# generic-ebpf/generic-ebpf

Measured on AMD Instinct MI355X. Metric: Mpkt/s device-resident (64-insn filter, 64B pkts); achieved HBM GB/s vs peak, higher is better.
Workload: dtype u64; 1 GPU; c4; desc=64-insn classify + array-map lookup, 64 B packets, packets_total=67108864, packets_per_gpu=67108864, packet_bytes=64, prog_slots=553, dprog_entries=122, variant=0, exec=compiled, kernel_layout=staged64, parallelism=dp1, launch=eager, faulted_packets=0

## Files before the change

### generic-ebpf_amd/csrc/asm/gen_interp.py

```python
#!/usr/bin/env python3
import os
import re
import sys

NREG = 11
_NT = int(os.environ.get("EBPF_ASM_NT", "3"))
ST_POLICY = " nt" if _NT & 1 else ""
LD_POLICY = " nt" if _NT & 2 else ""
PROBE_POLICY = ""
for _v, _n in (("EBPF_ASM_STPOL", "ST_POLICY"), ("EBPF_ASM_LDPOL", "LD_POLICY"),
               ("EBPF_ASM_PROBEPOL", "PROBE_POLICY")):
    if os.environ.get(_v):
        _p = os.environ[_v].replace("+", " ")
        globals()[_n] = "" if _p == "none" else " " + _p
PKT0 = 22
V_PKT = 38
V_LEN = 40
V_T = 41
V_STK = 42
V_L16 = 43
V_IDX = 43
V_RES = 44
H = [46, 47, 48, 49, 50, 51]
R = list(range(52, 63))
# ... 4 lines not shown
assert RETK_STAGED in (1, 2, 4, 8)


STAGED_IMAGE = True

HIST_REPLICAS = 8
HIST_REPLICA_BYTES = 257 * 8
HIST_TICKET_OFF = HIST_REPLICAS * HIST_REPLICA_BYTES


def set_retk(k):
    global RETK, V_RB, NVGPR, SLOTS
    RETK = k
    V_RB = 44 if RETK == 1 else 64
    NVGPR = 64 if RETK == 1 else 64 + 2 * RETK
    SLOTS = 16 if RETK == 8 else RETK


set_retk(RETK_STAGED)

S_CB = 4
S_ENT = 8
S_ALIVE = 16
S_SAVE = 18
S_PROG, S_MAPS, S_DATA, S_OFFS, S_OFFBASE, S_RET, S_FAULTS, S_HIST = 20, 22, 24, 26, 28, 30, 32, 34
S_COUNT, S_STRIDE, S_START, S_NMAPS, S_NENT = 36, 38, 39, 40, 41
S_STKSTRIDE, S_LDSBASE = 42, 43
S_GROUP, S_GSTRIDE, S_NGROUPS, S_PKTLDS = 44, 45, 46, 47
S_MASK = 48
S_LINK = 50
S_CODE = 52
# ... 161 lines not shown
def mode_set(bit):
    return "s_or_b32 %s, %s, %s" % (s(S_MODE), s(S_MODE), "%d" % (1 << bit) if bit < 4 else "0x%x" % (1 << bit))


VF_OVERLAY = 0
VF_VSTORE = 1
VF_EXTENTS = 2
VF_KEEP = 3
VF_WCAP = 4
VF_ENTRIES_SHIFT, VF_ENTRIES_BITS = 8, 8
PKTLDS_HDRSTAGE = 31
PKTLDS_HDRKEEP = 30
WAVES_SB_SHIFT = 28
HIST_STORE = 0
WPHASE_PERIOD_SHIFT = 16
WPHASE_WIDE = 31

LOOP_BUDGET = 1 << 20
OVL_COUNT, VST_SCRATCH, WCOUNT, OVL_ENTRIES = 4, 8, 16, 24
WRITES_MAX = 16
FAULT_WRITES = 11


def variants(arity):
    if arity == 3:
        return [(d, o) for o in range(64) for d in range(NREG)]
    if arity == 2:
        return [(d, s) for d in range(NREG) for s in range(NREG)]
    if arity == 1:
        return [(d, None) for d in range(NREG)]
    return [(None, None)]
# ... 1743 lines not shown
              "s_mov_b64 exec, vcc",
              "s_mov_b32 m0, s67",
              "s_nop 0",
              "global_load_lds_dwordx4 %s, s[64:65]%s" % (v(H[4]), LD_POLICY)]
        if qq < 3:
            L += ["s_add_u32 s64, s64, 1024", "s_addc_u32 s65, s65, 0",
                  "s_add_u32 s67, s67, 1024"]
    L += [".Lpf_ret:",
          "s_setpc_b64 %s" % sp(S_LINK)]
    return L


def kernel(name, staged, jit=False):
    k = "K%s%s" % ("s" if staged else "g", "j" if jit else "")
    L = [".globl %s" % name, ".p2align 8", ".type %s,@function" % name, "%s:" % name]
    if name == "ebpf_jit_s64" and phased() and SLOTS == 16:
        L += [".globl ebpf_jit_s64w", ".type ebpf_jit_s64w,@function", "ebpf_jit_s64w:"]
    L += ["v_readfirstlane_b32 %s, v0" % s(S_WAVE),
          "s_lshr_b32 %s, %s, 6" % (s(S_WAVE), s(S_WAVE)),
          "s_load_dwordx16 s[%d:%d], %s" % (S_PROG, S_PROG + 15, karg_regs(
              ("prog", S_PROG), ("maps", S_MAPS), ("data", S_DATA), ("offsets", S_OFFS),
              ("off_base", S_OFFBASE), ("ret", S_RET), ("faults", S_FAULTS), ("hist", S_HIST))),
          "s_load_dwordx8 s[%d:%d], %s" % (S_COUNT, S_COUNT + 7, karg_regs(
              ("count", S_COUNT), ("stride", S_STRIDE), ("start", S_START), ("nmaps", S_NMAPS),
              ("nentries", S_NENT), ("stack_stride", S_STKSTRIDE), ("lds_stack_base", S_LDSBASE))),
          "s_load_dword %s, %s" % (s(S_GSTRIDE), karg("total_waves")),
          "s_load_dword %s, %s" % (s(S_PKTLDS), karg("lds_pkt_base")),
          "s_mov_b64 %s, src_shared_base" % sp(S_SHARED),
          "v_mov_b32 v%d, 0x00010203" % V_SEL,
          "s_getpc_b64 %s" % sp(S_CB),
          ".L%s_pc:" % k,
          "s_add_u32 %s, %s, .Lcb-.L%s_pc" % (s(S_CB), s(S_CB), k),
# ... 95 lines not shown


def ret_slot_write(x0, x1):
    return ["v_mov_b32 v%d, %s" % (V_RES, x0), "v_mov_b32 v%d, %s" % (V_RES + 1, x1)]


def phased():
    return STAGED_IMAGE and RETK > 1


def slot_commit():
    if RETK == 1:
        return []
    L = ["s_mov_b64 exec, -1",
         "s_and_b32 %s, %s, %s" % (s(S_BYTES), s(S_GROUP), s(S_KMASK))]
    if phased() and SLOTS == 16:
        L += ["s_cmp_eq_u32 %s, 0" % s(S_BYTES),
              "s_cbranch_scc0 .Lsc_half",
              "s_bitcmp1_b32 %s, %d" % (s(S_WPHASE), WPHASE_WIDE),
              "s_cbranch_scc0 .Lsc_half",
              "s_xor_b32 %s, %s, 0x80000000" % (s(S_PEND), s(S_PEND)),
              ".Lsc_half:",
              "s_lshr_b32 %s, %s, 28" % (s(S_T0), s(S_PEND)),
              "s_and_b32 %s, %s, 8" % (s(S_T0), s(S_T0)),
              "s_or_b32 %s, %s, %s" % (s(S_BYTES), s(S_BYTES), s(S_T0)),
              "s_bitset1_b32 %s, %s" % (s(S_PEND), s(S_BYTES))]
    elif phased():
        L.append("s_bitset1_b32 %s, %s" % (s(S_PEND), s(S_BYTES)))
    return L + [
            "s_lshl_b32 %s, %s, 1" % (s(S_BYTES), s(S_BYTES)),
            "s_set_gpr_idx_on %s, gpr_idx(DST)" % s(S_BYTES),
            "v_mov_b32 v%d, v%d" % (V_RB, V_RES),
            "v_mov_b32 v%d, v%d" % (V_RB + 1, V_RES + 1),
            "s_set_gpr_idx_off"]


def store_phased(tag, final):
    P = s(S_PEND)
    L = ["s_cmp_eq_u32 %s, 0" % s(S_WPHASE),
         "s_cbranch_scc1 .Lph_off_%s" % tag] + (
        ["s_waitcnt lgkmcnt(0)"] if not final else []) + [
         "s_and_b32 %s, %s, 0xffff" % (s(S_T0), P),
         "s_cbranch_scc0 .Lsp_none_%s" % tag]
    if not final:
        L += [
              "s_and_b32 %s, %s, %s" % (s(S_T0), s(S_GROUP), s(S_KMASK)),
              "s_lshr_b32 %s, %s, 28" % (s(S_T1), P),
              "s_and_b32 %s, %s, 8" % (s(S_T1), s(S_T1)),
              "s_cmp_eq_u32 %s, 0" % s(S_T0),
              "s_cbranch_scc0 .Lph_nf_%s" % tag,
              "s_bitcmp1_b32 %s, %d" % (s(S_WPHASE), WPHASE_WIDE),
              "s_cbranch_scc0 .Lph_nf_%s" % tag,
              "s_xor_b32 %s, %s, 8" % (s(S_T1), s(S_T1)),
              ".Lph_nf_%s:" % tag,
              "s_or_b32 %s, %s, %s" % (s(S_T0), s(S_T0), s(S_T1)),
              "s_bitcmp1_b32 %s, %s" % (P, s(S_T0)),
              "s_cbranch_scc1 .Lph_write_%s" % tag,
              "s_and_b32 %s, %s, 0x%x" % (s(S_T1), s(S_WPHASE), 0x1f << WPHASE_PERIOD_SHIFT),
              "s_and_b32 %s, %s, 0xffff" % (s(S_T2), s(S_WPHASE)),
              "s_bfe_u32 %s, %s, %s" % (s(S_T0), s(S_CLOCK), s(S_T1)),
              "s_cmp_lt_u32 %s, %s" % (s(S_T0), s(S_T2)),
              "s_cbranch_scc0 .Lsp_none_%s" % tag,
              ".Lph_write_%s:" % tag]
    L += ["s_mov_b64 exec, -1",
          "v_lshrrev_b32 %s, 1, v%d" % (v(R[0]), V_L16),
          "s_andn2_b32 %s, %s, %s" % (s(S_T1), s(S_PREVG), s(S_KMASK)),
          "s_add_u32 %s, %s, %s" % (s(S_T2), s(S_GSTRIDE), s(S_KMASK)),
          "s_sub_u32 %s, %s, %s" % (s(S_T0), s(S_T1), s(S_T2)),
          "s_bitcmp1_b32 %s, %d" % (s(S_WPHASE), WPHASE_WIDE),
          "s_cselect_b32 %s, %s, 0" % (s(S_T2), s(S_T2)),
          "s_sub_u32 %s, %s, %s" % (s(S_T2), s(S_T0), s(S_T2)),
          "s_and_b32 %s, %s, %s" % (s(S_T3), s(S_PREVG), s(S_KMASK)),
          "s_lshr_b32 s66, %s, 6" % s(S_COUNT),
          "s_add_u32 s67, %s, %s" % (s(S_T1), s(S_KMASK)),
          "s_cmp_lt_u32 s67, s66",
          "s_cbranch_scc0 .Lph_ragged_%s" % tag]
    for lo, g in ((60, S_T1), (62, S_T0), (64, S_T2)):
        L += ["s_lshl_b32 s%d, %s, 9" % (lo, s(g)),
              "s_lshr_b32 s%d, %s, 23" % (lo + 1, s(g)),
              "s_add_u32 s%d, s%d, %s" % (lo, lo, s(S_RET)),
              "s_addc_u32 s%d, s%d, %s" % (lo + 1, lo + 1, s(S_RET + 1))]
    halves = [0] if RETK == SLOTS else [0, 1]

    def slots_of(half, ragged):
        out = []
        for own in (True, False):
            h = half if own else 1 - half
            if h not in halves:
                continue
            for i in range(RETK):
                j = 8 * h + i
                sk = ".Lph_%s%d_%d_%s" % ("r" if ragged else "f", half, j, tag)
                out += ["s_bitcmp1_b32 %s, %d" % (P, j), "s_cbranch_scc0 %s" % sk]
                if not ragged:
                    if own:
                        out += ["s_cmp_ge_u32 %s, %d" % (s(S_T3), i),
                                "s_cselect_b64 s[66:67], s[60:61], s[64:65]"]
                    out.append("global_store_dwordx2 %s, v[%d:%d], s[%d:%d] offset:%d%s" % (
                        v(R[0]), V_RB + 2 * j, V_RB + 2 * j + 1, 66 if own else 62,
                        67 if own else 63, 512 * i, ST_POLICY))
                else:
                    if own:
                        out += ["s_cmp_ge_u32 %s, %d" % (s(S_T3), i),
                                "s_cselect_b32 %s, %s, %s" % (s(S_BYTES), s(S_T1), s(S_T2))]
                    else:
                        out.append("s_mov_b32 %s, %s" % (s(S_BYTES), s(S_T0)))
                    out += ["s_add_u32 %s, %s, %d" % (s(S_BYTES), s(S_BYTES), i),
                            "s_lshl_b32 s66, %s, 6" % s(S_BYTES),
                            "s_sub_u32 s66, %s, s66" % s(S_COUNT),
                            "v_cmp_gt_u32_e64 vcc, s66, %s" % v(R[1]),
                            "s_mov_b64 exec, vcc",
                            "s_lshl_b32 s66, %s, 9" % s(S_BYTES),
                            "s_lshr_b32 s67, %s, 23" % s(S_BYTES),
                            "s_add_u32 s66, s66, %s" % s(S_RET),
                            "s_addc_u32 s67, s67, %s" % s(S_RET + 1),
                            "global_store_dwordx2 %s, v[%d:%d], s[66:67]%s" % (
                                v(R[0]), V_RB + 2 * j, V_RB + 2 * j + 1, ST_POLICY),
                            "s_mov_b64 exec, -1"]
                out.append(sk + ":")
        return out

    for ragged in (False, True):
        if ragged:
            L += [".Lph_ragged_%s:" % tag,
                  "v_lshrrev_b32 %s, 4, v%d" % (v(R[1]), V_L16)]
        if len(halves) > 1:
            L += ["s_bitcmp1_b32 %s, 31" % P,
                  "s_cbranch_scc1 .Lph_%sh1_%s" % ("r" if ragged else "f", tag)]
        L += slots_of(0, ragged) + ["s_branch .Lph_done_%s" % tag]
        if len(halves) > 1:
            L += [".Lph_%sh1_%s:" % ("r" if ragged else "f", tag)] + slots_of(1, ragged) + [
                  "s_branch .Lph_done_%s" % tag]
    L += [".Lph_done_%s:" % tag,
          "s_and_b32 %s, %s, 0x80000000" % (P, P),
          "s_branch .Lsp_none_%s" % tag,
          ".Lph_off_%s:" % tag]
    return L


def store_prev_results(tag, final):
    L = store_phased(tag, final) if phased() else []
    L += ["s_cmp_eq_u32 %s, -1" % s(S_PREVG),
         "s_cbranch_scc1 .Lsp_none_%s" % tag]
    if not final and RETK > 1:
        L += ["s_and_b32 %s, %s, %s" % (s(S_T0), s(S_PREVG), s(S_KMASK)),
              "s_cmp_lg_u32 %s, %s" % (s(S_T0), s(S_KMASK)),
              "s_cbranch_scc1 .Lsp_none_%s" % tag]
    L += ["s_mov_b64 exec, -1",
          "s_andn2_b32 %s, %s, %s" % (s(S_T0), s(S_PREVG), s(S_KMASK)) if RETK > 1 else
# ... 522 lines not shown
             ("L16", V_L16), ("RES", V_RES), ("GIDX", V_GIDX), ("HVAL", V_HVAL), ("SEL", V_SEL)]
    vregs += [("H%d" % i, r) for i, r in enumerate(H)] + [("R%d" % i, r) for i, r in enumerate(R)]
    out += ["#define AH_S_%s %d" % x for x in sregs] + ["#define AH_V_%s %d" % x for x in vregs]
    out += ["// bits of the mode word s[AH_S_MODE]"]
    out += ["#define AH_MODE_%s %d" % x for x in (
        ("STAGED", MODE_STAGED), ("JIT", MODE_JIT), ("STRUCTURED", MODE_STRUCTURED),
        ("HDRSTAGE", MODE_HDRSTAGE), ("OVERLAY", MODE_OVERLAY), ("KEEP", MODE_KEEP),
        ("EXTENTS", MODE_EXTENTS))]
    out += ["// dprog.h / ebpf_gpu.h values the kernels were generated with; asm_runtime.cpp asserts them"]
    values = (
        ("DP_VF_OVERLAY", 1 << VF_OVERLAY), ("DP_VF_VSTORE", 1 << VF_VSTORE),
        ("DP_VF_EXTENTS", 1 << VF_EXTENTS), ("DP_VF_KEEP", 1 << VF_KEEP), ("DP_VF_WCAP", 1 << VF_WCAP),
        ("DP_VF_ENTRIES_SHIFT", VF_ENTRIES_SHIFT), ("DP_VF_ENTRIES_MAX", (1 << VF_ENTRIES_BITS) - 1),
        ("DP_PKTLDS_HDRSTAGE", 1 << PKTLDS_HDRSTAGE), ("DP_PKTLDS_HDRKEEP", 1 << PKTLDS_HDRKEEP),
        ("DP_WAVES_SB_SHIFT", WAVES_SB_SHIFT), ("DP_HIST_STORE", 1 << HIST_STORE),
        ("DP_WPHASE_PERIOD_SHIFT", WPHASE_PERIOD_SHIFT), ("DP_WPHASE_WIDE", 1 << WPHASE_WIDE),
        ("DP_LOOP_BUDGET", LOOP_BUDGET), ("DP_OVL_COUNT", OVL_COUNT), ("DP_OVL_SCRATCH", VST_SCRATCH),
        ("DP_WCOUNT", WCOUNT), ("DP_OVL_ENTRIES", OVL_ENTRIES), ("DP_WRITES_MAX", WRITES_MAX),
        ("EBPF_FAULT_WRITES", FAULT_WRITES), ("DP_HIST_REPLICAS", HIST_REPLICAS),
        ("DP_HIST_REPLICA_BYTES", HIST_REPLICA_BYTES), ("DP_HIST_TICKET_OFF", HIST_TICKET_OFF),
        ("DP_HIST_PARTIAL_BYTES", HIST_TICKET_OFF + 64 * (HIST_REPLICAS + 1)))
    out += ["#define AH_%s %du" % x for x in values]
    out += ["#define AH_SHARED_VALUES(X) " + " ".join("X(%s)" % n for n, _ in values)]
    out += ["// ebpf_jit_tmpl's entries, in the table's order"]
    jt = [re.sub(r"^(\.Ljt_|\.Lr_|\.L|ebpf_)", "", n).upper() for n in JT_LABELS] + ["AREA_BYTES"]
    out += ["enum {"] + ["\tAH_JT_%s," % n for n in jt] + ["\tAH_JT_COUNT", "};"]
    out += ["#define AH_JIT_ENTRY_OFF %d  // a compiled program's start block in ebpf_jit_area" % JIT_ENTRY_OFF]
    return out


NSGPR_INTERP = S_JOIN
# ... 10 lines not shown
                                     (out_s0, 1, False, False),
                                     (out_s3, RETK_INTERP, True, True)):
        set_retk(k)
        INTERP_IMAGE = interp
        if not staged:
            NVGPR += GEN_HOIST_REGS
        h = generate(out_s, staged)
        header = header or h
        assert h[:-2] == header[:-2]
    header = header[:-2] + ["#define AH_RET_GROUPS_STAGED %d  // groups per result burst, staged kernels"
                            % RETK_STAGED,
                            "#define AH_NVGPR_STAGED %d" % (64 if RETK_STAGED == 1 else 64 + 2 * RETK_STAGED),
                            "#define AH_RET_GROUPS_GENERAL 1",
                            "#define AH_NVGPR_STAGED_WIDE %d  // ebpf_jit_s64w: 16 result slots "
                            "(write phasing), 0 = none" % (96 if RETK_STAGED == 8 else 0),
                            "#define AH_NVGPR_GENERAL %d" % (64 + GEN_HOIST_REGS),
                            "#define AH_NVGPR_INTERP %d  // the interpreter's staged image (m3)"
                            % (64 if RETK_INTERP == 1 else 64 + 2 * RETK_INTERP),
                            "#define AH_RET_GROUPS_INTERP %d" % RETK_INTERP]
    with open(out_h, "w") as f:
        f.write("\n".join(header) + "\n")


def header_families():
    classes = []
    for _, _, cls, _ in FAMILIES:
        if cls not in classes:
            classes.append(cls)
    for cls in classes:
        idx = [i for _, _, c, i in FAMILIES if c == cls]
# ... 92 lines not shown
    header.append("#define AH_S_RUNMASK %d  // general image: s[76:77], a hoisted-load run's lanes" % S_RUNMASK)
    header.append("#define AH_V_IDX %d  // general image: the lane's packet index" % V_IDX)
    header.append("#define AH_RET_GROUPS %d" % RETK)
    header.append("#define AH_NVGPR %d" % NVGPR)
    A += link_kernel()
    A += [".p2align 2", ".Lhandler_table:"]
    A += ["  .long %s-.Llink_base" % lab for lab in table]
    A += [".p2align 2", "ebpf_jit_meta:"] + meta
    A += jit_templates()
    A += [".p2align 8", "ebpf_jit_area:", "  .fill %d, 4, 0xbf810000" % (JIT_AREA_BYTES // 4)]
    vtop = 0
    for ln in A:
        code = ln.split(";")[0].split("//")[0]
        for a, b, c in re.findall(r"\bv(\d+)\b|\bv\[(\d+):(\d+)\]", code):
            vtop = max(vtop, int(a or c))
    vwide = V_RB + 2 * SLOTS if (staged_image and SLOTS == 16) else NVGPR
    assert vtop < max(NVGPR, vwide), "image code uses v%d, the kernels allocate %d VGPRs" % (
        vtop, max(NVGPR, vwide))
    kernarg = 232
    nsg = NSGPR_STAGED if (staged_image or GEN_JOIN) else NSGPR_GEN
    if INTERP_IMAGE:
        top = 0
        for ln in A:
            for a, b, c in re.findall(r"\bs(\d+)\b|\bs\[(\d+):(\d+)\]", ln.split(";")[0].split("//")[0]):
                top = max(top, int(a or c))
        assert top < NSGPR_INTERP, "interpreter image uses s%d" % top
    ks = [("ebpf_interp_s64", kernarg, 0, NVGPR, NSGPR_INTERP if INTERP_IMAGE else nsg, 256),
          ("ebpf_interp_gen", kernarg, 0, NVGPR, nsg, 256),
          ("ebpf_jit_s64", kernarg, 0, NVGPR, nsg, 256),
          ("ebpf_jit_gen", kernarg, 0, NVGPR, nsg, 256),
          ("ebpf_asm_link", 16, 0, 16, 16, 64)]
    if vwide > NVGPR:
        ks.append(("ebpf_jit_s64w", kernarg, 0, vwide, nsg, 256))
    for name, ka, lds, vg, sg, wg in ks:
        A += kd(name, lds, vg, sg, ka, wg)
    md = metadata(ks)
    with open(out_s, "w") as f:
        f.write("\n".join(("\t" + x if not (x.endswith(":") or x.startswith(".") or x.startswith(" ")) else x)
                          for x in A) + "\n")
        f.write("\n".join(md) + "\n")
    return header


if __name__ == "__main__":
    main()
```

### generic-ebpf_amd/csrc/dprog.h

```cpp
#pragma once
#include <stdint.h>
#include <stddef.h>

enum dp_kind : uint16_t {
	DK_FAULT = 0x100,
	DK_CALL_LOOKUP = 0x101,
	DK_MOV64R = 0x102,
	DK_NEG64 = 0x103,
	DK_NEG32 = 0x104,
	DK_ARSH64I = 0x105,
	DK_ARSH64R = 0x106,
	DK_ARSH32I = 0x107,
	DK_ARSH32R = 0x108,
	DK_DIV64Z = 0x109,
	DK_MOD64Z = 0x10a,
	DK_DIV32Z = 0x10b,
	DK_MOD32Z = 0x10c,
	DK_CALL_UPDATE = 0x10d,
	DK_LOOPINIT = 0x10e,
	DK_LOOPCNT = 0x10f,
	DK_CALL_HDELETE = 0x110,
	DK_CNT_STORE = 0x111,
	DK_XADD = 0x112,
	DK_OVLINIT = 0x113,
};
#define DP_VF_OVERLAY 1u
#define DP_VF_VSTORE 2u
#define DP_VF_EXTENTS 4u
#define DP_VF_KEEP 8u
#define DP_VF_WCAP 16u
#define DP_VF_ENTRIES_SHIFT 8u
#define DP_VF_ENTRIES_MAX 255u
#define DP_PKTLDS_HDRSTAGE 0x80000000u
#define DP_PKTLDS_HDRKEEP 0x40000000u
#define DP_WAVES_SB_SHIFT 28u
#define DP_HIST_STORE 1u
#define DP_WPHASE_PERIOD_SHIFT 16u
#define DP_WPHASE_WIDE 0x80000000u
#define DP_AUX_SIZE 0xffu
#define DP_AUX_FETCH 0x100u
#define DP_AUX_IMM 0x200u
#define DP_AUX_SYNTH 1u
#define DP_AUX_DELETE 1u
#define DP_LOOP_BUDGET (1u << 20)
#define DP_CLS_JMP32 6

struct dp_entry {
	uint64_t handler;
	uint64_t imm;
	uint32_t next;
	uint32_t target;
	uint16_t kind;
	uint8_t dst, src;
// ... 94 lines not shown
```

### generic-ebpf_amd/csrc/host/asm_jit.cpp

```cpp
#include <elf.h>
#include <hip/hip_runtime.h>

#include "asm_cc.h"
#include "asm_handlers.h"
#include "gfx950_enc.h"
#include "runtime.h"

int asm_lower(const dprog_host &xl, int mode, const std::vector<dp_map> &table,
	      std::vector<dp_entry> &out, uint32_t *stack_stride, std::string *err);

namespace {

static_assert(AH_S_OPND == 10 && AH_JT_MOV_S11 == AH_JT_MOV_S10 + 1 && AH_JT_MOV_S12 == AH_JT_MOV_S10 + 2 &&
		      AH_JT_MOV_S13 == AH_JT_MOV_S10 + 3 && AH_JT_MOV_S14 == AH_JT_MOV_S10 + 4 &&
		      AH_JT_MOV_S15 == AH_JT_MOV_S10 + 5,
	      "the s_mov templates of the operand registers s10..s15 are consecutive");

struct jit_image {
	bool ok = false;
	std::string why;
	size_t cb = 0;
	std::vector<uint32_t> body_off, body_len;
	uint32_t t[AH_JT_COUNT] = {};
};
// ... 564 lines not shown
		}
		memcpy(&img[area + pos[e]], g.data(), g.size());
	}
	if (structured) {
		g.clear();
		G.long_jump(T[AH_JT_GROUP_DONE]);
		memcpy(&img[area + end_pos], g.data(), g.size());
	}
	if (code)
		code->assign(img.begin() + area, img.begin() + area + total);
	return 0;
}

int
asm_jit_build(int device, const dprog_host &xl, int mode, const std::vector<dp_map> &table,
	      void **mod_out, void **fn_out, void **fn_wide_out, uint32_t *stack_stride,
	      std::string *err)
{
	std::vector<unsigned char> img;
	int e = asm_jit_emit(xl, mode, table, &img, nullptr, stack_stride, err);
	if (e)
		return e;
	if (hipSetDevice(device) != hipSuccess)
		return EIO;
	hipModule_t mod = nullptr;
	if (hipModuleLoadData(&mod, img.data()) != hipSuccess) {
		*err = "loading the compiled program failed";
		return EIO;
	}
	hipFunction_t fn = nullptr;
	if (hipModuleGetFunction(&fn, mod, mode == 1 ? "ebpf_jit_s64" : "ebpf_jit_gen") != hipSuccess) {
		hipModuleUnload(mod);
		*err = "compiled program kernel missing";
		return EIO;
	}
	hipFunction_t fw = nullptr;
	if (fn_wide_out && mode == 1 && AH_NVGPR_STAGED_WIDE &&
	    hipModuleGetFunction(&fw, mod, "ebpf_jit_s64w") != hipSuccess)
		fw = nullptr;
	*mod_out = mod;
	*fn_out = fn;
	if (fn_wide_out)
		*fn_wide_out = fw;
	return 0;
}

void
asm_jit_release(void *mod)
{
	if (mod)
		hipModuleUnload(static_cast<hipModule_t>(mod));
}
```

### generic-ebpf_amd/csrc/host/asm_runtime.cpp

```cpp
#include <cstdio>
#include <hip/hip_runtime.h>

#include <algorithm>

#include "asm_handlers.h"
#include "runtime.h"

extern "C" hipError_t hipExtModuleLaunchKernel(hipFunction_t f, uint32_t gx, uint32_t gy, uint32_t gz,
					       uint32_t lx, uint32_t ly, uint32_t lz, size_t shared,
					       hipStream_t stream, void **params, void **extra,
					       hipEvent_t start, hipEvent_t stop, uint32_t flags);

#define X(member, off) \
	static_assert(offsetof(dp_launch, member) == off, \
		      "dp_launch." #member " is not where the kernels load it: " #off);
AH_LAUNCH_FIELDS(X)
#undef X
static_assert(sizeof(dp_launch) == AH_KERNARG_BYTES, "dp_launch is the kernels' argument block");
static_assert(offsetof(dp_map, handle) == AH_M_HANDLE && offsetof(dp_map, dev_base) == AH_M_DEV_BASE &&
		      offsetof(dp_map, value_size) == AH_M_VALUE_SIZE &&
		      offsetof(dp_map, max_entries) == AH_M_MAX_ENTRIES &&
		      offsetof(dp_map, lds_off) == AH_M_LDS_OFF && offsetof(dp_map, flags) == AH_M_FLAGS &&
		      sizeof(dp_map) == AH_MAP_REC_BYTES,
	      "dp_map is loaded whole into the kernels' record registers");
// ... 747 lines not shown
		lo = std::min(lo, x.handler);
		hi = std::max(hi, x.handler);
	}
	for (const dp_entry &x : back)
		if (x.handler == 0 || (x.handler & 3) || hi - lo > asm_image_len(mode)) {
			hipFree(d);
			*err = "handler link produced implausible addresses";
			return EIO;
		}
	*d_out = d;
	return 0;
}

hipError_t
launch_interp_asm(const dp_launch &L0, hipStream_t stream, int device, int mode,
		  uint32_t map_lds_bytes, void *fn, void *fn_wide, uint32_t stream_cap, hipEvent_t ev_start,
		  hipEvent_t ev_stop, unsigned long long *user_hist, bool hist_overwrite)
{
	asm_module *mod = module_for(device);
	if (!mod->ok)
		return hipErrorNotSupported;
	const uint64_t chunk = 1ull << 28;
	for (uint64_t c0 = 0; c0 < L0.count; c0 += chunk) {
		dp_launch L = L0;
		L.count = (L0.count - c0 < chunk) ? L0.count - c0 : chunk;
		if (L0.offsets)
			L.offsets = L0.offsets + ((L0.vflags & DP_VF_EXTENTS) ? 2 * c0 : c0);
		else
			L.data = L0.data + c0 * L0.stride;
		L.ret = L0.ret + c0;
		L.pkt_base = L0.pkt_base + c0;
		if (L0.faults)
// ... 32 lines not shown
		uint32_t sb = retk;
		if (interp_staged)
			sb = kInterpSuperblock;
		if (const char *ks = getenv("EBPF_SUPERBLOCK"))
			while (sb > 1 && (uint32_t)atoi(ks) < sb)
				sb >>= 1;
		uint64_t wgs = (groups + 4 * sb - 1) / (4 * sb);
		if (wgs > cap)
			wgs = cap;
		uint32_t log2k = 0;
		while ((1u << log2k) < sb)
			log2k++;
		L.total_waves = (uint32_t)(wgs * 4) | (log2k << DP_WAVES_SB_SHIFT);
		L.wphase = 0;
		if (mode == 1 && !interp_staged && sb > 1 && stream_cap == kStreamWorkgroups &&
		    groups >= 2 * sb * 4 * wgs)
			L.wphase = fn_wide ? (DP_WPHASE_WIDE | (12u << DP_WPHASE_PERIOD_SHIFT) | 1024u)
					   : ((11u << DP_WPHASE_PERIOD_SHIFT) | 640u);
		if (const char *wp = getenv("EBPF_WPHASE")) {
			unsigned bits = 0, win = 0, slots = 8;
			const int nf = sscanf(wp, "%u,%u,%u", &bits, &win, &slots);
			L.wphase = (nf >= 2 && bits >= 4 && bits <= 20 && win < (1u << bits))
				       ? ((bits << DP_WPHASE_PERIOD_SHIFT) | win) : 0u;
			if (L.wphase && slots == 16 && fn_wide)
				L.wphase |= DP_WPHASE_WIDE;
			if (!(mode == 1 && !interp_staged && sb > 1))
				L.wphase = 0;
		}
		if ((L.wphase & DP_WPHASE_WIDE) && fn_wide && AH_NVGPR_STAGED_WIDE) {
			const uint64_t wide_cap = (uint64_t)mod->cus * std::min<uint32_t>(
				wg_per_cu, 512 / ((AH_NVGPR_STAGED_WIDE + 7) & ~7));
			if (wgs > wide_cap) {
				wgs = wide_cap;
				L.total_waves = (uint32_t)(wgs * 4) | (log2k << DP_WAVES_SB_SHIFT);
			}
		}
		L.hist_user = user_hist;
		L.hist_flags = (hist_overwrite && c0 == 0) ? DP_HIST_STORE : 0u;
		L.nwg = (uint32_t)wgs;
		size_t sz = sizeof(L);
		void *extra[] = {HIP_LAUNCH_PARAM_BUFFER_POINTER, &L, HIP_LAUNCH_PARAM_BUFFER_SIZE, &sz,
				 HIP_LAUNCH_PARAM_END};
		hipFunction_t k = fn ? static_cast<hipFunction_t>((L.wphase & DP_WPHASE_WIDE) ? fn_wide : fn)
				     : (mode == 1 ? mod->k_staged : mod->k_general);
		if (L.hist && !L.hist_rows)
			return hipErrorInvalidValue;
		const bool single = c0 == 0 && L0.count <= chunk;
		hipError_t e;
		if (single && ev_start && ev_stop) {
			e = hipExtModuleLaunchKernel(k, (uint32_t)wgs * 256u, 1, 1, 256, 1, 1, lds, stream,
						     nullptr, extra, ev_start, ev_stop, 0);
		} else {
			if (ev_start && c0 == 0)
				hipEventRecord(ev_start, stream);
			e = hipModuleLaunchKernel(k, (unsigned)wgs, 1, 1, 256, 1, 1, lds, stream, nullptr,
						  extra);
			if (e == hipSuccess && ev_stop && c0 + chunk >= L0.count)
				hipEventRecord(ev_stop, stream);
// ... 30 lines not shown
```

### generic-ebpf_amd/csrc/host/gpu_runtime.cpp

```cpp
#include <chrono>

#include "runtime.h"

namespace {

uint32_t
plan_map_lds(const struct ebpf_map *em, uint32_t *used)
{
	if (em->is_hashtable())
		return ~0u;
	const uint64_t bytes = (uint64_t)em->value_size * em->max_entries;
	if (bytes == 0 || bytes % 4 != 0 || *used + bytes > kMapLdsBudget)
		return ~0u;
	const uint32_t off = kMapLdsBase + *used;
	*used += (uint32_t)((bytes + 15) & ~15ull);
	return off;
}

dp_map
map_record(const struct ebpf_map *em, uint32_t *lds_used)
{
	const map_device_layout l = map_device_layout_of(em);
	dp_map m;
	memset(&m, 0, sizeof(m));
// ... 167 lines not shown
	return 0;
}

static int
jit_entries(struct ebpf_prog *ep, dprog_device *dp, int mode)
{
	std::lock_guard<std::mutex> g(ep->dlock);
	if (dp->jit_fn[mode])
		return 0;
	if (dp->jit_err[mode])
		return dp->jit_err[mode];
	std::string msg;
	const auto t0 = std::chrono::steady_clock::now();
	int err = asm_jit_build(dp->device, *ep->xlated, mode, dp->table, &dp->jit_mod[mode],
				&dp->jit_fn[mode], mode == 1 ? &dp->jit_fn_wide : nullptr,
				&dp->jit_stride[mode], &msg);
	dp->build_ms[mode] =
	    std::chrono::duration<double, std::milli>(std::chrono::steady_clock::now() - t0).count();
	if (err) {
		dp->jit_err[mode] = err;
		return fail(err, msg);
	}
	return 0;
}

static int
asm_entries(struct ebpf_prog *ep, dprog_device *dp, int mode)
{
	std::lock_guard<std::mutex> g(ep->dlock);
	if (dp->d_asm[mode])
// ... 93 lines not shown
		unsigned long long *user_hist = L.hist;
		if (L.hist) {
			void *part = nullptr;
			if ((err = rows_acquire(dp->device, stream, &part)))
				return fail(err, "no verdict-partial buffer");
			L.hist_rows = static_cast<uint32_t *>(part);
			L.hist = static_cast<unsigned long long *>(part);
		}
		bool hash = false;
		for (const dp_map &m : dp->table)
			hash = hash || (m.flags & DP_MAP_HASH) != 0;
		uint32_t wg_cap = 0;
		if (mode == 1 && fn)
			wg_cap = (hash || ep->xlated->has_loops) ? kProbeWorkgroups : kStreamWorkgroups;
		e = launch_interp_asm(L, stream, dp->device, mode, dp->map_lds_bytes, fn,
				      fn ? dp->jit_fn_wide : nullptr, wg_cap, ev_start, ev_stop, user_hist,
				      hist_overwrite);
	} else {
		L.prog = dp->d_entries;
		dp->last_exec = EBPF_EXEC_HIP;
		dp->last_layout = 0;
		if (hist_overwrite && L.hist &&
		    (e = hipMemsetAsync(L.hist, 0, EBPF_HIST_BINS * sizeof(uint64_t), stream)) !=
			hipSuccess)
			return hip_fail(e, "hipMemsetAsync(hist)");
		if (spill) {
			const uint64_t per = 16ull * ep->xlated->ovl_entries;
			uint64_t chunk = std::max<uint64_t>(256, ((1ull << 30) / per) & ~255ull);
			chunk = std::min<uint64_t>(chunk, std::max<uint64_t>(L.count, 1));
			uint8_t *buf = nullptr;
			if ((err = ovl_acquire(dp->device, stream, chunk * per, &buf)))
// ... 240 lines not shown
```

### generic-ebpf_amd/csrc/host/internal.h

```cpp
#pragma once

#include <errno.h>
#include <stdint.h>
#include <stdlib.h>
#include <string.h>

#include <atomic>
#include <memory>
#include <mutex>
#include <set>
#include <string>
#include <vector>

#include "ebpf.h"
#include "ebpf_gpu.h"
#include "ebpf_vm_isa.h"
#include "../dprog.h"
#include "map_writes.h"

#define EBPF_EXPORT extern "C" __attribute__((visibility("default")))

enum ebpf_obj_type_id : uint32_t { EBPF_OBJ_TYPE_PROG = 0, EBPF_OBJ_TYPE_MAP = 1 };

struct ebpf_env {
// ... 74 lines not shown

struct dprog_device {
	int device = -1;
	dp_entry *d_entries = nullptr;
	dp_map *d_maps = nullptr;
	std::vector<dp_map> table;
	uint32_t nentries = 0;
	uint32_t nmaps = 0;
	uint32_t map_lds_bytes = 0;
	dp_entry *d_asm[kModes] = {};
	uint32_t asm_stride[kModes] = {};
	int asm_err[kModes] = {};
	void *jit_mod[kModes] = {};
	void *jit_fn[kModes] = {};
	void *jit_fn_wide = nullptr;
	uint32_t jit_stride[kModes] = {};
	int jit_err[kModes] = {};
	double build_ms[kModes] = {};
	void *d_upd = nullptr;
	std::vector<struct upd_map> upd_host;
	uint64_t win_words = 0;
	uint32_t upd_stride = 0;
	int last_exec = -1;
	int last_layout = -1;
};

struct dprog_host;
bool prog_writes_maps(const dprog_host &xl);

enum av_kind : uint8_t {
// ... 86 lines not shown
```

### generic-ebpf_amd/csrc/host/runtime.h

```cpp
#pragma once
#include <hip/hip_runtime.h>

#include <algorithm>

#include "internal.h"

int fail(int err, const std::string &msg);
int hip_fail(hipError_t e, const char *what);
int device_count();
void take_time_events(hipEvent_t *start, hipEvent_t *stop);

inline bool
in_list(const std::vector<uint16_t> &v, size_t t)
{
	return std::find(v.begin(), v.end(), (uint16_t)t) != v.end();
}

struct rows_slot;
struct upd_owner {
	rows_slot *slot = nullptr;
	unsigned long long sid = 0;
};
int rows_acquire(int device, hipStream_t stream, void **out);
int ovl_acquire(int device, hipStream_t stream, size_t bytes, uint8_t **out);
// ... 41 lines not shown
int upd_plan_for(struct ebpf_prog *ep, dprog_device *dp, uint64_t count, hipStream_t stream, upd_plan *P);
int upd_fetch(const dprog_device *dp, const upd_plan &P, hipStream_t stream, uint64_t first, host_log *out);
int upd_apply_host(struct ebpf_prog *ep, const std::vector<host_log> &logs, bool arrays);
int delta_merge_host(struct ebpf_prog *ep, int ndev, const int *devices);
int upd_finish(struct ebpf_prog *ep, dprog_device *dp, const upd_plan &P, hipStream_t stream);

int prepare(struct ebpf_prog *ep, int device, dprog_device **out);
int launch(struct ebpf_prog *ep, dprog_device *dp, const dp_launch &L0, hipStream_t stream,
	   hipEvent_t ev_start = nullptr, hipEvent_t ev_stop = nullptr, bool hist_overwrite = false,
	   upd_plan *plan = nullptr);
int validate_batch(const struct ebpf_pkt_batch *b, uint32_t allowed_flags = 0);
int check_device(int device);

hipError_t launch_interp_v0(const dp_launch &L, hipStream_t stream);
hipError_t launch_interp_asm(const dp_launch &L, hipStream_t stream, int device, int mode,
			     uint32_t map_lds_bytes, void *fn, void *fn_wide, uint32_t stream_cap,
			     hipEvent_t ev_start, hipEvent_t ev_stop, unsigned long long *user_hist,
			     bool hist_overwrite);
int asm_available(int device);
bool asm_lds_fits(int mode, uint32_t map_lds_bytes, uint32_t stack_stride);
bool asm_program_needs_general(const dprog_host &xl);
bool asm_program_stores_last(const dprog_host &xl);
bool asm_program_gstage(const dprog_host &xl);
bool asm_program_hdrlds(const dprog_host &xl);
bool asm_hdrlds_fits(uint32_t map_lds_bytes, uint32_t stack_stride);
int asm_build_entries(int device, const dprog_host &xl, int mode, const std::vector<dp_map> &table,
		      dp_entry **d_out, uint32_t *stack_stride, std::string *err);
int asm_jit_build(int device, const dprog_host &xl, int mode, const std::vector<dp_map> &table,
		  void **mod_out, void **fn_out, void **fn_wide_out, uint32_t *stack_stride, std::string *err);
void asm_jit_release(void *mod);
int asm_jit_emit(const dprog_host &xl, int mode, const std::vector<dp_map> &table,
		 std::vector<unsigned char> *img_out, std::vector<unsigned char> *code,
		 uint32_t *stack_stride, std::string *err);
int rccl_hist_allreduce(int ndev, const int *devices, uint64_t *const *hist, hipStream_t *streams,
			std::string *msg);
```

Before: 87880 Mpkt/s.

## Add 32-slot result write phasing kernel variant for staged JIT

Extends the write-phasing scheme for result stores from 16 to 32 buffered result slots, organised as four rotating quarters tracked by a cursor field in the wphase word. A new ebpf_jit_s64x entry point with 128 VGPRs is emitted and selected by the host when there are enough groups, using a longer period and window. The aim is to batch more result writes into larger, less frequent bursts to reduce HBM write interference. The cost is higher VGPR pressure, which caps workgroups per CU and lowers occupancy, plus more scalar bookkeeping per commit.

```diff
diff --git a/generic-ebpf_amd/csrc/asm/gen_interp.py b/generic-ebpf_amd/csrc/asm/gen_interp.py
--- a/generic-ebpf_amd/csrc/asm/gen_interp.py
+++ b/generic-ebpf_amd/csrc/asm/gen_interp.py
@@ -42,7 +42,7 @@
     RETK = k
     V_RB = 44 if RETK == 1 else 64
     NVGPR = 64 if RETK == 1 else 64 + 2 * RETK
-    SLOTS = 16 if RETK == 8 else RETK
+    SLOTS = 32 if RETK == 8 else RETK
 
 
 set_retk(RETK_STAGED)
@@ -234,7 +234,10 @@
 WAVES_SB_SHIFT = 28
 HIST_STORE = 0
 WPHASE_PERIOD_SHIFT = 16
-WPHASE_WIDE = 31
+WPHASE_CUR_SHIFT = 24
+WPHASE_HQ_SHIFT = 30
+WPHASE_WIDE = 1 << WPHASE_HQ_SHIFT
+WPHASE_X32 = 3 << WPHASE_HQ_SHIFT
 
 LOOP_BUDGET = 1 << 20
 OVL_COUNT, VST_SCRATCH, WCOUNT, OVL_ENTRIES = 4, 8, 16, 24
@@ -2008,8 +2011,9 @@
 def kernel(name, staged, jit=False):
     k = "K%s%s" % ("s" if staged else "g", "j" if jit else "")
     L = [".globl %s" % name, ".p2align 8", ".type %s,@function" % name, "%s:" % name]
-    if name == "ebpf_jit_s64" and phased() and SLOTS == 16:
-        L += [".globl ebpf_jit_s64w", ".type ebpf_jit_s64w,@function", "ebpf_jit_s64w:"]
+    if name == "ebpf_jit_s64" and phased() and SLOTS > RETK:
+        L += [".globl ebpf_jit_s64w", ".type ebpf_jit_s64w,@function", "ebpf_jit_s64w:",
+              ".globl ebpf_jit_s64x", ".type ebpf_jit_s64x,@function", "ebpf_jit_s64x:"]
     L += ["v_readfirstlane_b32 %s, v0" % s(S_WAVE),
           "s_lshr_b32 %s, %s, 6" % (s(S_WAVE), s(S_WAVE)),
           "s_load_dwordx16 s[%d:%d], %s" % (S_PROG, S_PROG + 15, karg_regs(
@@ -2135,15 +2139,17 @@
         return []
     L = ["s_mov_b64 exec, -1",
          "s_and_b32 %s, %s, %s" % (s(S_BYTES), s(S_GROUP), s(S_KMASK))]
-    if phased() and SLOTS == 16:
+    if phased() and SLOTS > RETK:
         L += ["s_cmp_eq_u32 %s, 0" % s(S_BYTES),
-              "s_cbranch_scc0 .Lsc_half",
-              "s_bitcmp1_b32 %s, %d" % (s(S_WPHASE), WPHASE_WIDE),
-              "s_cbranch_scc0 .Lsc_half",
-              "s_xor_b32 %s, %s, 0x80000000" % (s(S_PEND), s(S_PEND)),
-              ".Lsc_half:",
-              "s_lshr_b32 %s, %s, 28" % (s(S_T0), s(S_PEND)),
-              "s_and_b32 %s, %s, 8" % (s(S_T0), s(S_T0)),
+              "s_cbranch_scc0 .Lsc_quarter",
+              "s_lshr_b32 %s, %s, %d" % (s(S_T0), s(S_WPHASE), WPHASE_HQ_SHIFT),
+              "s_lshl_b32 %s, %s, %d" % (s(S_T0), s(S_T0), WPHASE_CUR_SHIFT),
+              "s_or_b32 %s, %s, 0x%x" % (s(S_T0), s(S_T0), 0xffffffff & ~(7 << WPHASE_CUR_SHIFT)),
+              "s_add_u32 %s, %s, 0x%x" % (s(S_WPHASE), s(S_WPHASE), 1 << WPHASE_CUR_SHIFT),
+              "s_and_b32 %s, %s, %s" % (s(S_WPHASE), s(S_WPHASE), s(S_T0)),
+              ".Lsc_quarter:",
+              "s_bfe_u32 %s, %s, 0x%x" % (s(S_T0), s(S_WPHASE), 2 << 16 | WPHASE_CUR_SHIFT),
+              "s_lshl_b32 %s, %s, %d" % (s(S_T0), s(S_T0), RETK.bit_length() - 1),
               "s_or_b32 %s, %s, %s" % (s(S_BYTES), s(S_BYTES), s(S_T0)),
               "s_bitset1_b32 %s, %s" % (s(S_PEND), s(S_BYTES))]
     elif phased():
@@ -2158,22 +2164,23 @@
 
 def store_phased(tag, final):
     P = s(S_PEND)
+    cur_field = 2 << 16 | WPHASE_CUR_SHIFT
     L = ["s_cmp_eq_u32 %s, 0" % s(S_WPHASE),
          "s_cbranch_scc1 .Lph_off_%s" % tag] + (
         ["s_waitcnt lgkmcnt(0)"] if not final else []) + [
-         "s_and_b32 %s, %s, 0xffff" % (s(S_T0), P),
-         "s_cbranch_scc0 .Lsp_none_%s" % tag]
+         "s_cmp_eq_u32 %s, 0" % P,
+         "s_cbranch_scc1 .Lsp_none_%s" % tag]
     if not final:
         L += [
               "s_and_b32 %s, %s, %s" % (s(S_T0), s(S_GROUP), s(S_KMASK)),
-              "s_lshr_b32 %s, %s, 28" % (s(S_T1), P),
-              "s_and_b32 %s, %s, 8" % (s(S_T1), s(S_T1)),
+              "s_bfe_u32 %s, %s, 0x%x" % (s(S_T1), s(S_WPHASE), cur_field),
               "s_cmp_eq_u32 %s, 0" % s(S_T0),
               "s_cbranch_scc0 .Lph_nf_%s" % tag,
-              "s_bitcmp1_b32 %s, %d" % (s(S_WPHASE), WPHASE_WIDE),
-              "s_cbranch_scc0 .Lph_nf_%s" % tag,
-              "s_xor_b32 %s, %s, 8" % (s(S_T1), s(S_T1)),
+              "s_add_u32 %s, %s, 1" % (s(S_T1), s(S_T1)),
+              "s_lshr_b32 %s, %s, %d" % (s(S_T2), s(S_WPHASE), WPHASE_HQ_SHIFT),
+              "s_and_b32 %s, %s, %s" % (s(S_T1), s(S_T1), s(S_T2)),
               ".Lph_nf_%s:" % tag,
+              "s_lshl_b32 %s, %s, %d" % (s(S_T1), s(S_T1), RETK.bit_length() - 1),
               "s_or_b32 %s, %s, %s" % (s(S_T0), s(S_T0), s(S_T1)),
               "s_bitcmp1_b32 %s, %s" % (P, s(S_T0)),
               "s_cbranch_scc1 .Lph_write_%s" % tag,
@@ -2187,73 +2194,72 @@
           "v_lshrrev_b32 %s, 1, v%d" % (v(R[0]), V_L16),
           "s_andn2_b32 %s, %s, %s" % (s(S_T1), s(S_PREVG), s(S_KMASK)),
           "s_add_u32 %s, %s, %s" % (s(S_T2), s(S_GSTRIDE), s(S_KMASK)),
-          "s_sub_u32 %s, %s, %s" % (s(S_T0), s(S_T1), s(S_T2)),
-          "s_bitcmp1_b32 %s, %d" % (s(S_WPHASE), WPHASE_WIDE),
-          "s_cselect_b32 %s, %s, 0" % (s(S_T2), s(S_T2)),
-          "s_sub_u32 %s, %s, %s" % (s(S_T2), s(S_T0), s(S_T2)),
           "s_and_b32 %s, %s, %s" % (s(S_T3), s(S_PREVG), s(S_KMASK)),
+          "s_bfe_u32 s68, %s, 0x%x" % (s(S_WPHASE), cur_field),
+          "s_lshr_b32 s69, %s, %d" % (s(S_WPHASE), WPHASE_HQ_SHIFT),
+          "s_add_u32 %s, s69, 1" % s(S_BYTES),
+          "s_mul_i32 %s, %s, %s" % (s(S_BYTES), s(S_BYTES), s(S_T2)),
           "s_lshr_b32 s66, %s, 6" % s(S_COUNT),
           "s_add_u32 s67, %s, %s" % (s(S_T1), s(S_KMASK)),
           "s_cmp_lt_u32 s67, s66",
           "s_cbranch_scc0 .Lph_ragged_%s" % tag]
-    for lo, g in ((60, S_T1), (62, S_T0), (64, S_T2)):
-        L += ["s_lshl_b32 s%d, %s, 9" % (lo, s(g)),
-              "s_lshr_b32 s%d, %s, 23" % (lo + 1, s(g)),
-              "s_add_u32 s%d, s%d, %s" % (lo, lo, s(S_RET)),
-              "s_addc_u32 s%d, s%d, %s" % (lo + 1, lo + 1, s(S_RET + 1))]
-    halves = [0] if RETK == SLOTS else [0, 1]
-
-    def slots_of(half, ragged):
-        out = []
-        for own in (True, False):
-            h = half if own else 1 - half
-            if h not in halves:
-                continue
-            for i in range(RETK):
-                j = 8 * h + i
-                sk = ".Lph_%s%d_%d_%s" % ("r" if ragged else "f", half, j, tag)
-                out += ["s_bitcmp1_b32 %s, %d" % (P, j), "s_cbranch_scc0 %s" % sk]
-                if not ragged:
-                    if own:
-                        out += ["s_cmp_ge_u32 %s, %d" % (s(S_T3), i),
-                                "s_cselect_b64 s[66:67], s[60:61], s[64:65]"]
-                    out.append("global_store_dwordx2 %s, v[%d:%d], s[%d:%d] offset:%d%s" % (
-                        v(R[0]), V_RB + 2 * j, V_RB + 2 * j + 1, 66 if own else 62,
-                        67 if own else 63, 512 * i, ST_POLICY))
-                else:
-                    if own:
-                        out += ["s_cmp_ge_u32 %s, %d" % (s(S_T3), i),
-                                "s_cselect_b32 %s, %s, %s" % (s(S_BYTES), s(S_T1), s(S_T2))]
-                    else:
-                        out.append("s_mov_b32 %s, %s" % (s(S_BYTES), s(S_T0)))
-                    out += ["s_add_u32 %s, %s, %d" % (s(S_BYTES), s(S_BYTES), i),
-                            "s_lshl_b32 s66, %s, 6" % s(S_BYTES),
-                            "s_sub_u32 s66, %s, s66" % s(S_COUNT),
-                            "v_cmp_gt_u32_e64 vcc, s66, %s" % v(R[1]),
-                            "s_mov_b64 exec, vcc",
-                            "s_lshl_b32 s66, %s, 9" % s(S_BYTES),
-                            "s_lshr_b32 s67, %s, 23" % s(S_BYTES),
-                            "s_add_u32 s66, s66, %s" % s(S_RET),
-                            "s_addc_u32 s67, s67, %s" % s(S_RET + 1),
-                            "global_store_dwordx2 %s, v[%d:%d], s[66:67]%s" % (
-                                v(R[0]), V_RB + 2 * j, V_RB + 2 * j + 1, ST_POLICY),
-                            "s_mov_b64 exec, -1"]
-                out.append(sk + ":")
-        return out
-
+    lg = RETK.bit_length() - 1
+
+    def quarter(h, ragged):
+        rf = "r" if ragged else "f"
+        out = ["s_bfe_u32 s66, %s, 0x%x" % (P, RETK << 16 | RETK * h),
+               "s_cbranch_scc0 .Lph_%sq%d_%s" % (rf, h, tag),
+               "s_sub_u32 s64, s68, %d" % h,
+               "s_and_b32 s64, s64, s69",
+               "s_mul_i32 s65, s64, %s" % s(S_T2),
+               "s_sub_u32 %s, %s, s65" % (s(S_T0), s(S_T1)),
+               "s_cmp_eq_u32 s64, 0",
+               "s_cselect_b32 s65, %s, 0" % s(S_BYTES),
+               "s_cselect_b32 s64, %s, %d" % (s(S_T3), RETK - 1),
+               "s_sub_u32 s65, %s, s65" % s(S_T0)]
+        if not ragged:
+            for lo, g in ((60, s(S_T0)), (62, "s65")):
+                out += ["s_lshl_b32 s%d, %s, 9" % (lo, g),
+                        "s_lshr_b32 s%d, %s, 23" % (lo + 1, g),
+                        "s_add_u32 s%d, s%d, %s" % (lo, lo, s(S_RET)),
+                        "s_addc_u32 s%d, s%d, %s" % (lo + 1, lo + 1, s(S_RET + 1))]
+        for i in range(RETK):
+            j = RETK * h + i
+            sk = ".Lph_%s%d_%s" % (rf, j, tag)
+            out += ["s_bitcmp1_b32 %s, %d" % (P, j), "s_cbranch_scc0 %s" % sk,
+                    "s_cmp_ge_u32 s64, %d" % i]
+            if not ragged:
+                out += ["s_cselect_b64 s[66:67], s[60:61], s[62:63]",
+                        "global_store_dwordx2 %s, v[%d:%d], s[66:67] offset:%d%s" % (
+                            v(R[0]), V_RB + 2 * j, V_RB + 2 * j + 1, 512 * i, ST_POLICY)]
+            else:
+                out += ["s_cselect_b32 s66, %s, s65" % s(S_T0),
+                        "s_add_u32 s66, s66, %d" % i,
+                        "s_lshl_b32 s67, s66, 6",
+                        "s_sub_u32 s67, %s, s67" % s(S_COUNT),
+                        "v_cmp_gt_u32_e64 vcc, s67, %s" % v(R[1]),
+                        "s_mov_b64 exec, vcc",
+                        "s_lshr_b32 s67, s66, 23",
+                        "s_lshl_b32 s66, s66, 9",
+                        "s_add_u32 s66, s66, %s" % s(S_RET),
+                        "s_addc_u32 s67, s67, %s" % s(S_RET + 1),
+                        "global_store_dwordx2 %s, v[%d:%d], s[66:67]%s" % (
+                            v(R[0]), V_RB + 2 * j, V_RB + 2 * j + 1, ST_POLICY),
+                        "s_mov_b64 exec, -1"]
+            out.append(sk + ":")
+        return out + [".Lph_%sq%d_%s:" % (rf, h, tag)]
+
+    assert 1 << lg == RETK and SLOTS % RETK == 0 and SLOTS <= 32
     for ragged in (False, True):
         if ragged:
             L += [".Lph_ragged_%s:" % tag,
                   "v_lshrrev_b32 %s, 4, v%d" % (v(R[1]), V_L16)]
-        if len(halves) > 1:
-            L += ["s_bitcmp1_b32 %s, 31" % P,
-                  "s_cbranch_scc1 .Lph_%sh1_%s" % ("r" if ragged else "f", tag)]
-        L += slots_of(0, ragged) + ["s_branch .Lph_done_%s" % tag]
-        if len(halves) > 1:
-            L += [".Lph_%sh1_%s:" % ("r" if ragged else "f", tag)] + slots_of(1, ragged) + [
-                  "s_branch .Lph_done_%s" % tag]
+        for h in range(SLOTS // RETK):
+            L += quarter(h, ragged)
+        if not ragged:
+            L.append("s_branch .Lph_done_%s" % tag)
     L += [".Lph_done_%s:" % tag,
-          "s_and_b32 %s, %s, 0x80000000" % (P, P),
+          "s_mov_b32 %s, 0" % P,
           "s_branch .Lsp_none_%s" % tag,
           ".Lph_off_%s:" % tag]
     return L
@@ -2806,7 +2812,8 @@
         ("DP_VF_ENTRIES_SHIFT", VF_ENTRIES_SHIFT), ("DP_VF_ENTRIES_MAX", (1 << VF_ENTRIES_BITS) - 1),
         ("DP_PKTLDS_HDRSTAGE", 1 << PKTLDS_HDRSTAGE), ("DP_PKTLDS_HDRKEEP", 1 << PKTLDS_HDRKEEP),
         ("DP_WAVES_SB_SHIFT", WAVES_SB_SHIFT), ("DP_HIST_STORE", 1 << HIST_STORE),
-        ("DP_WPHASE_PERIOD_SHIFT", WPHASE_PERIOD_SHIFT), ("DP_WPHASE_WIDE", 1 << WPHASE_WIDE),
+        ("DP_WPHASE_PERIOD_SHIFT", WPHASE_PERIOD_SHIFT), ("DP_WPHASE_WIDE", WPHASE_WIDE),
+        ("DP_WPHASE_X32", WPHASE_X32),
         ("DP_LOOP_BUDGET", LOOP_BUDGET), ("DP_OVL_COUNT", OVL_COUNT), ("DP_OVL_SCRATCH", VST_SCRATCH),
         ("DP_WCOUNT", WCOUNT), ("DP_OVL_ENTRIES", OVL_ENTRIES), ("DP_WRITES_MAX", WRITES_MAX),
         ("EBPF_FAULT_WRITES", FAULT_WRITES), ("DP_HIST_REPLICAS", HIST_REPLICAS),
@@ -2847,6 +2854,8 @@
                             "#define AH_RET_GROUPS_GENERAL 1",
                             "#define AH_NVGPR_STAGED_WIDE %d  // ebpf_jit_s64w: 16 result slots "
                             "(write phasing), 0 = none" % (96 if RETK_STAGED == 8 else 0),
+                            "#define AH_NVGPR_STAGED_X32 %d  // ebpf_jit_s64x: 32 result slots, 0 = none"
+                            % (128 if RETK_STAGED == 8 else 0),
                             "#define AH_NVGPR_GENERAL %d" % (64 + GEN_HOIST_REGS),
                             "#define AH_NVGPR_INTERP %d  // the interpreter's staged image (m3)"
                             % (64 if RETK_INTERP == 1 else 64 + 2 * RETK_INTERP),
@@ -2969,9 +2978,10 @@
         code = ln.split(";")[0].split("//")[0]
         for a, b, c in re.findall(r"\bv(\d+)\b|\bv\[(\d+):(\d+)\]", code):
             vtop = max(vtop, int(a or c))
-    vwide = V_RB + 2 * SLOTS if (staged_image and SLOTS == 16) else NVGPR
-    assert vtop < max(NVGPR, vwide), "image code uses v%d, the kernels allocate %d VGPRs" % (
-        vtop, max(NVGPR, vwide))
+    vwide = V_RB + 4 * RETK if (staged_image and SLOTS > RETK) else NVGPR
+    vx32 = V_RB + 2 * SLOTS if (staged_image and SLOTS > RETK) else NVGPR
+    assert vtop < max(NVGPR, vx32), "image code uses v%d, the kernels allocate %d VGPRs" % (
+        vtop, max(NVGPR, vx32))
     kernarg = 232
     nsg = NSGPR_STAGED if (staged_image or GEN_JOIN) else NSGPR_GEN
     if INTERP_IMAGE:
@@ -2987,6 +2997,7 @@
           ("ebpf_asm_link", 16, 0, 16, 16, 64)]
     if vwide > NVGPR:
         ks.append(("ebpf_jit_s64w", kernarg, 0, vwide, nsg, 256))
+        ks.append(("ebpf_jit_s64x", kernarg, 0, vx32, nsg, 256))
     for name, ka, lds, vg, sg, wg in ks:
         A += kd(name, lds, vg, sg, ka, wg)
     md = metadata(ks)
diff --git a/generic-ebpf_amd/csrc/dprog.h b/generic-ebpf_amd/csrc/dprog.h
--- a/generic-ebpf_amd/csrc/dprog.h
+++ b/generic-ebpf_amd/csrc/dprog.h
@@ -36,7 +36,8 @@
 #define DP_WAVES_SB_SHIFT 28u
 #define DP_HIST_STORE 1u
 #define DP_WPHASE_PERIOD_SHIFT 16u
-#define DP_WPHASE_WIDE 0x80000000u
+#define DP_WPHASE_WIDE 0x40000000u
+#define DP_WPHASE_X32 0xc0000000u
 #define DP_AUX_SIZE 0xffu
 #define DP_AUX_FETCH 0x100u
 #define DP_AUX_IMM 0x200u
diff --git a/generic-ebpf_amd/csrc/host/asm_jit.cpp b/generic-ebpf_amd/csrc/host/asm_jit.cpp
--- a/generic-ebpf_amd/csrc/host/asm_jit.cpp
+++ b/generic-ebpf_amd/csrc/host/asm_jit.cpp
@@ -602,7 +602,7 @@
 
 int
 asm_jit_build(int device, const dprog_host &xl, int mode, const std::vector<dp_map> &table,
-	      void **mod_out, void **fn_out, void **fn_wide_out, uint32_t *stack_stride,
+	      void **mod_out, void **fn_out, void **fn_wide_out, void **fn_x32_out, uint32_t *stack_stride,
 	      std::string *err)
 {
 	std::vector<unsigned char> img;
@@ -626,10 +626,16 @@
 	if (fn_wide_out && mode == 1 && AH_NVGPR_STAGED_WIDE &&
 	    hipModuleGetFunction(&fw, mod, "ebpf_jit_s64w") != hipSuccess)
 		fw = nullptr;
+	hipFunction_t fx = nullptr;
+	if (fn_x32_out && mode == 1 && AH_NVGPR_STAGED_X32 &&
+	    hipModuleGetFunction(&fx, mod, "ebpf_jit_s64x") != hipSuccess)
+		fx = nullptr;
 	*mod_out = mod;
 	*fn_out = fn;
 	if (fn_wide_out)
 		*fn_wide_out = fw;
+	if (fn_x32_out)
+		*fn_x32_out = fx;
 	return 0;
 }
 
diff --git a/generic-ebpf_amd/csrc/host/asm_runtime.cpp b/generic-ebpf_amd/csrc/host/asm_runtime.cpp
--- a/generic-ebpf_amd/csrc/host/asm_runtime.cpp
+++ b/generic-ebpf_amd/csrc/host/asm_runtime.cpp
@@ -785,8 +785,8 @@
 
 hipError_t
 launch_interp_asm(const dp_launch &L0, hipStream_t stream, int device, int mode,
-		  uint32_t map_lds_bytes, void *fn, void *fn_wide, uint32_t stream_cap, hipEvent_t ev_start,
-		  hipEvent_t ev_stop, unsigned long long *user_hist, bool hist_overwrite)
+		  uint32_t map_lds_bytes, void *fn, void *fn_wide, void *fn_x32, uint32_t stream_cap,
+		  hipEvent_t ev_start, hipEvent_t ev_stop, unsigned long long *user_hist, bool hist_overwrite)
 {
 	asm_module *mod = module_for(device);
 	if (!mod->ok)
@@ -849,22 +849,30 @@
 		L.total_waves = (uint32_t)(wgs * 4) | (log2k << DP_WAVES_SB_SHIFT);
 		L.wphase = 0;
 		if (mode == 1 && !interp_staged && sb > 1 && stream_cap == kStreamWorkgroups &&
-		    groups >= 2 * sb * 4 * wgs)
+		    groups >= 2 * sb * 4 * wgs) {
 			L.wphase = fn_wide ? (DP_WPHASE_WIDE | (12u << DP_WPHASE_PERIOD_SHIFT) | 1024u)
 					   : ((11u << DP_WPHASE_PERIOD_SHIFT) | 640u);
+			if (fn_x32 && groups >= 4 * sb * 4 * wgs)
+				L.wphase = DP_WPHASE_X32 | (13u << DP_WPHASE_PERIOD_SHIFT) | 2048u;
+		}
 		if (const char *wp = getenv("EBPF_WPHASE")) {
 			unsigned bits = 0, win = 0, slots = 8;
 			const int nf = sscanf(wp, "%u,%u,%u", &bits, &win, &slots);
-			L.wphase = (nf >= 2 && bits >= 4 && bits <= 20 && win < (1u << bits))
+			L.wphase = (nf >= 2 && bits >= 4 && bits <= 20 && win < (1u << bits) && win <= 0xffffu)
 				       ? ((bits << DP_WPHASE_PERIOD_SHIFT) | win) : 0u;
 			if (L.wphase && slots == 16 && fn_wide)
 				L.wphase |= DP_WPHASE_WIDE;
+			if (L.wphase && slots == 32 && fn_x32)
+				L.wphase |= DP_WPHASE_X32;
 			if (!(mode == 1 && !interp_staged && sb > 1))
 				L.wphase = 0;
 		}
-		if ((L.wphase & DP_WPHASE_WIDE) && fn_wide && AH_NVGPR_STAGED_WIDE) {
+		const bool x32 = (L.wphase & DP_WPHASE_X32) == DP_WPHASE_X32 && fn_x32 && AH_NVGPR_STAGED_X32;
+		const bool wide = !x32 && (L.wphase & DP_WPHASE_WIDE) && fn_wide && AH_NVGPR_STAGED_WIDE;
+		if (x32 || wide) {
+			const uint32_t nv = x32 ? AH_NVGPR_STAGED_X32 : AH_NVGPR_STAGED_WIDE;
 			const uint64_t wide_cap = (uint64_t)mod->cus * std::min<uint32_t>(
-				wg_per_cu, 512 / ((AH_NVGPR_STAGED_WIDE + 7) & ~7));
+				wg_per_cu, 512 / ((nv + 7) & ~7));
 			if (wgs > wide_cap) {
 				wgs = wide_cap;
 				L.total_waves = (uint32_t)(wgs * 4) | (log2k << DP_WAVES_SB_SHIFT);
@@ -876,7 +884,7 @@
 		size_t sz = sizeof(L);
 		void *extra[] = {HIP_LAUNCH_PARAM_BUFFER_POINTER, &L, HIP_LAUNCH_PARAM_BUFFER_SIZE, &sz,
 				 HIP_LAUNCH_PARAM_END};
-		hipFunction_t k = fn ? static_cast<hipFunction_t>((L.wphase & DP_WPHASE_WIDE) ? fn_wide : fn)
+		hipFunction_t k = fn ? static_cast<hipFunction_t>(x32 ? fn_x32 : wide ? fn_wide : fn)
 				     : (mode == 1 ? mod->k_staged : mod->k_general);
 		if (L.hist && !L.hist_rows)
 			return hipErrorInvalidValue;
diff --git a/generic-ebpf_amd/csrc/host/gpu_runtime.cpp b/generic-ebpf_amd/csrc/host/gpu_runtime.cpp
--- a/generic-ebpf_amd/csrc/host/gpu_runtime.cpp
+++ b/generic-ebpf_amd/csrc/host/gpu_runtime.cpp
@@ -205,6 +205,7 @@
 	const auto t0 = std::chrono::steady_clock::now();
 	int err = asm_jit_build(dp->device, *ep->xlated, mode, dp->table, &dp->jit_mod[mode],
 				&dp->jit_fn[mode], mode == 1 ? &dp->jit_fn_wide : nullptr,
+				mode == 1 ? &dp->jit_fn_x32 : nullptr,
 				&dp->jit_stride[mode], &msg);
 	dp->build_ms[mode] =
 	    std::chrono::duration<double, std::milli>(std::chrono::steady_clock::now() - t0).count();
@@ -328,7 +329,8 @@
 		if (mode == 1 && fn)
 			wg_cap = (hash || ep->xlated->has_loops) ? kProbeWorkgroups : kStreamWorkgroups;
 		e = launch_interp_asm(L, stream, dp->device, mode, dp->map_lds_bytes, fn,
-				      fn ? dp->jit_fn_wide : nullptr, wg_cap, ev_start, ev_stop, user_hist,
+				      fn ? dp->jit_fn_wide : nullptr, fn ? dp->jit_fn_x32 : nullptr, wg_cap,
+				      ev_start, ev_stop, user_hist,
 				      hist_overwrite);
 	} else {
 		L.prog = dp->d_entries;
diff --git a/generic-ebpf_amd/csrc/host/internal.h b/generic-ebpf_amd/csrc/host/internal.h
--- a/generic-ebpf_amd/csrc/host/internal.h
+++ b/generic-ebpf_amd/csrc/host/internal.h
@@ -112,6 +112,7 @@
 	void *jit_mod[kModes] = {};
 	void *jit_fn[kModes] = {};
 	void *jit_fn_wide = nullptr;
+	void *jit_fn_x32 = nullptr;
 	uint32_t jit_stride[kModes] = {};
 	int jit_err[kModes] = {};
 	double build_ms[kModes] = {};
diff --git a/generic-ebpf_amd/csrc/host/runtime.h b/generic-ebpf_amd/csrc/host/runtime.h
--- a/generic-ebpf_amd/csrc/host/runtime.h
+++ b/generic-ebpf_amd/csrc/host/runtime.h
@@ -79,7 +79,7 @@
 
 hipError_t launch_interp_v0(const dp_launch &L, hipStream_t stream);
 hipError_t launch_interp_asm(const dp_launch &L, hipStream_t stream, int device, int mode,
-			     uint32_t map_lds_bytes, void *fn, void *fn_wide, uint32_t stream_cap,
+			     uint32_t map_lds_bytes, void *fn, void *fn_wide, void *fn_x32, uint32_t stream_cap,
 			     hipEvent_t ev_start, hipEvent_t ev_stop, unsigned long long *user_hist,
 			     bool hist_overwrite);
 int asm_available(int device);
@@ -92,7 +92,8 @@
 int asm_build_entries(int device, const dprog_host &xl, int mode, const std::vector<dp_map> &table,
 		      dp_entry **d_out, uint32_t *stack_stride, std::string *err);
 int asm_jit_build(int device, const dprog_host &xl, int mode, const std::vector<dp_map> &table,
-		  void **mod_out, void **fn_out, void **fn_wide_out, uint32_t *stack_stride, std::string *err);
+		  void **mod_out, void **fn_out, void **fn_wide_out, void **fn_x32_out, uint32_t *stack_stride,
+		  std::string *err);
 void asm_jit_release(void *mod);
 int asm_jit_emit(const dprog_host &xl, int mode, const std::vector<dp_map> &table,
 		 std::vector<unsigned char> *img_out, std::vector<unsigned char> *code,
```

New measurement: 88950 Mpkt/s, median of 6. +1.2%, better.
